# andreadiiorio/SpMV_openMP_CUDA

Measured on AMD Instinct MI355X. Metric: spmv_gflops, higher is better.
Workload: dtype f64

## Files before the change

spmv_openmp_cuda_amd/csrc/hip/tiles.hip:

```cpp
#include <hip/hip_runtime.h>
#include <cstring>
#include <cmath>
#include <chrono>
#include <rocprim/device/device_radix_sort.hpp>
#include <rocprim/device/device_scan.hpp>
#include <algorithm>
#include <vector>

#include "spmvHip.h"
#include "device_mat.hpp"

namespace spmvhip {

constexpr uint32_t PB_CBITS   = 14;
constexpr uint32_t PB_C       = 1u << PB_CBITS;
static_assert(PB_C % 1024 == 0 && PB_C * 8 <= 160 * 1024 && PB_C <= 65536, "slice width");
constexpr uint32_t PB_R_MAX   = 20000;
constexpr uint32_t PB_CUS_DEFAULT = 256;
constexpr uint32_t PB_CHUNK   = 1u << 17;
constexpr int      PB_THREADS = 1024;
constexpr uint32_t PD_WAVES   = 4;
constexpr int      PD_THREADS = PD_WAVES * 64;
constexpr size_t   PB_RESIDENT_BYTES = 288ull << 20;

struct BinMap {
    uint32_t n1 = 0, n2 = 0, a = 1, b = 1, c = 1;
    uint64_t z1 = 0, z2 = 0;
    __host__ __device__ uint32_t binOf(uint64_t row) const {
        return row < z1 ? (uint32_t)(row / a) : row < z2 ? n1 + (uint32_t)((row - z1) / b) : n1 + n2 + (uint32_t)((row - z2) / c);
    }
    __host__ __device__ uint64_t row0(uint32_t bin) const {
        return bin < n1 ? (uint64_t)bin * a : bin < n1 + n2 ? z1 + (uint64_t)(bin - n1) * b : z2 + (uint64_t)(bin - n1 - n2) * c;
    }
    __host__ __device__ uint32_t height(uint32_t bin) const { return bin < n1 ? a : bin < n1 + n2 ? b : c; }
    __host__ __device__ uint32_t maxHeight() const { uint32_t m = c; if (n1 && a > m) m = a; if (n2 && b > m) m = b; return m; }
};

struct TileFormat {
    uint32_t S = 0, B = 0, R = 0;
    BinMap    bins;
    uint64_t nnz = 0;
    void*     slab = nullptr;
    double*   val = nullptr;
    uint16_t* lcol = nullptr;
    uint16_t* lrow = nullptr;
    bool      det = false;
    uint32_t* pidx = nullptr;
    size_t    tempBytes = 0;
    uint2*    tl = nullptr;
    uint32_t  nList = 0;
    uint32_t* binPos = nullptr;
    uint32_t* waveTile = nullptr;
    uint3*    work = nullptr;
    uint32_t  nWork = 0;
    bool      ntStore = true;
    uint32_t* ready = nullptr;
    uint32_t* pushFail = nullptr;
    uint32_t  epoch = 0;
    uint32_t  cus = PB_CUS_DEFAULT;
    size_t    bytes = 0;
    spmvTilesOpts opts{0, 0, -1, 0, 0};
    uint32_t apiBins() const { return det ? (B + PD_WAVES - 1) / PD_WAVES : B; }
    uint32_t apiRows() const { return det ? PD_WAVES * bins.c : R; }
    BinMap   apiMap() const { if (!det) return bins; BinMap m; m.c = PD_WAVES * bins.c; return m; }
    uint32_t  chunk = 0;
    double    buildMs = 0;
    double    allocMs = 0;
    uint32_t* vmap = nullptr;
};

struct TileDst { double* p[SPMV_MAX_PEERS]; uint32_t n; };
struct TileSignal { uint32_t* ready; uint32_t epoch; };

namespace {

__device__ __forceinline__ uint64_t lin_block() { return (uint64_t)blockIdx.y * gridDim.x + blockIdx.x; }

struct PbPay { uint32_t vlo, vhi, row; };
static_assert(sizeof(PbPay) == 12 && alignof(PbPay) == 4, "payload layout");
__host__ __device__ __forceinline__ PbPay pb_pack(double v, uint32_t row) {
    uint64_t b;
    memcpy(&b, &v, 8);
    return PbPay{(uint32_t)b, (uint32_t)(b >> 32), row};
}
__host__ __device__ __forceinline__ double pb_value(const PbPay& e) {
    const uint64_t b = ((uint64_t)e.vhi << 32) | e.vlo;
    double v;
    memcpy(&v, &b, 8);
    return v;
}

template <typename I>
__global__ __launch_bounds__(256) void pb_payload_kernel(uint64_t M, const I* __restrict__ IRP, const uint32_t* __restrict__ JA,
                                                         const double* __restrict__ AS, uint32_t* __restrict__ keys,
                                                         PbPay* __restrict__ pay) {
    const uint64_t r = lin_block() * 4 + threadIdx.x / 64;
    if (r >= M) return;
    const uint64_t b = IRP[r], e = IRP[r + 1];
    for (uint64_t j = b + threadIdx.x % 64; j < e; j += 64) {
        const uint32_t c = JA[j];
        keys[j] = c;
        pay[j] = pb_pack(AS[j], (uint32_t)r);
    }
}

__global__ __launch_bounds__(256) void pb_bounds_kernel(
    uint64_t nnz, const PbPay* __restrict__ spay, const uint32_t* __restrict__ skeys,
    uint32_t B, BinMap bm, uint64_t nTiles, uint32_t* __restrict__ tileStart) {
    const uint64_t p = lin_block() * 256 + threadIdx.x;
    if (p >= nnz) return;
    const uint64_t t = (uint64_t)(skeys[p] >> PB_CBITS) * B + bm.binOf(spay[p].row);
    uint64_t tPrev;
    if (p == 0) tPrev = ~0ull;
    else tPrev = (uint64_t)(skeys[p - 1] >> PB_CBITS) * B + bm.binOf(spay[p - 1].row);
    if (t != tPrev)
        for (uint64_t u = tPrev + 1; u <= t; ++u) tileStart[u] = (uint32_t)p;
    if (p == nnz - 1)
        for (uint64_t u = t + 1; u <= nTiles; ++u) tileStart[u] = (uint32_t)nnz;
}

__global__ __launch_bounds__(256) void pb_lens_kernel(uint32_t S, uint32_t B, const uint32_t* __restrict__ tileStart,
                                                      uint32_t* __restrict__ lens, uint32_t* __restrict__ flags) {
    const uint64_t i = lin_block() * 256 + threadIdx.x;
    if (i >= (uint64_t)S * B) return;
    const uint32_t b = (uint32_t)(i / S), s = (uint32_t)(i % S);
    const uint64_t t = (uint64_t)s * B + b;
    const uint32_t len = tileStart[t + 1] - tileStart[t];
    lens[i] = len;
    flags[i] = len != 0;
}

__global__ __launch_bounds__(256) void pb_list_kernel(uint32_t S, uint32_t B, uint64_t nnz, const uint32_t* __restrict__ tileStart,
                                                      const uint32_t* __restrict__ lens, const uint32_t* __restrict__ bmStart,
                                                      const uint32_t* __restrict__ listIdx, uint32_t nList,
                                                      uint2* __restrict__ tl,
                                                      uint32_t* __restrict__ binPos, uint32_t* __restrict__ binTile) {
    const uint64_t i = lin_block() * 256 + threadIdx.x;
    if (i >= (uint64_t)S * B) return;
    const uint32_t b = (uint32_t)(i / S), s = (uint32_t)(i % S);
    if (lens[i]) {
        const uint64_t t = (uint64_t)s * B + b;
        tl[listIdx[i]] = make_uint2(bmStart[i], tileStart[t] - bmStart[i]);
    }
    if (s == 0) { binPos[b] = bmStart[i]; binTile[b] = listIdx[i]; }
    if (i + 1 == (uint64_t)S * B) { binPos[B] = (uint32_t)nnz; binTile[B] = nList; }
}

__global__ __launch_bounds__(256) void pb_place_kernel(
    uint64_t nnz, const PbPay* __restrict__ spay, const uint32_t* __restrict__ skeys,
    uint32_t S, uint32_t B, BinMap bm, const uint32_t* __restrict__ tileStart, const uint32_t* __restrict__ bmStart,
    double* __restrict__ val, uint16_t* __restrict__ lcol, uint16_t* __restrict__ lrow, uint32_t* __restrict__ pidx) {
    const uint64_t p = lin_block() * 256 + threadIdx.x;
    if (p >= nnz) return;
    const PbPay e = spay[p];
    const uint32_t key = skeys[p];
    const uint32_t bin = bm.binOf(e.row), slice = key >> PB_CBITS;
    val[p] = pb_value(e);
    lcol[p] = (uint16_t)(key & (PB_C - 1));
    const uint32_t within = (uint32_t)p - tileStart[(uint64_t)slice * B + bin];
    const uint32_t at = bmStart[(uint64_t)bin * S + slice] + within;
    lrow[at] = (uint16_t)(e.row - bm.row0(bin));
    if (pidx) pidx[at] = (uint32_t)p;
}

__global__ __launch_bounds__(256) void pb_fill_kernel(uint32_t* p, uint64_t n, uint32_t v) {
    const uint64_t i = lin_block() * 256 + threadIdx.x;
    if (i < n) p[i] = v;
}

__global__ __launch_bounds__(256) void pb_iota_kernel(uint64_t n, uint32_t* __restrict__ p) {
    const uint64_t i = lin_block() * 256 + threadIdx.x;
    if (i < n) p[i] = (uint32_t)i;
}
__global__ __launch_bounds__(256) void pb_invert_kernel(uint64_t n, const uint32_t* __restrict__ perm, uint32_t* __restrict__ inv) {
    const uint64_t p = lin_block() * 256 + threadIdx.x;
    if (p < n) inv[perm[p]] = (uint32_t)p;
}

typedef double   dbl2 __attribute__((ext_vector_type(2)));
typedef uint16_t ush2 __attribute__((ext_vector_type(2)));

constexpr int      P1_DEPTH = 8;
constexpr uint32_t P1_STEP  = 2 * PB_THREADS;
struct P1Regs { dbl2 a[P1_DEPTH]; ush2 c[P1_DEPTH]; };

template <bool UNIT>
__device__ __forceinline__ void p1_load(P1Regs& r, uint32_t p, uint32_t ve, const double* __restrict__ val,
                                        const uint16_t* __restrict__ lcol, double unitValue) {
#pragma unroll
    for (int u = 0; u < P1_DEPTH; ++u) {
        const uint32_t q = min(p + u * P1_STEP, ve - 2u);
        if (UNIT) r.a[u] = dbl2{unitValue, unitValue};
        else      r.a[u] = __builtin_nontemporal_load((const dbl2*)(val + q));
        r.c[u] = __builtin_nontemporal_load((const ush2*)(lcol + q));
    }
}

template <bool NT>
__device__ __forceinline__ void p1_store(const P1Regs& r, uint32_t p, uint32_t ve, const double* xs, double* __restrict__ prod) {
#pragma unroll
    for (int u = 0; u < P1_DEPTH; ++u) {
        const uint32_t q = p + u * P1_STEP;
        if (q < ve) {
            dbl2 o;
            o.x = r.a[u].x * xs[r.c[u].x]; o.y = r.a[u].y * xs[r.c[u].y];
            if (NT) __builtin_nontemporal_store(o, (dbl2*)(prod + q)); else *(dbl2*)(prod + q) = o;
        }
    }
}

template <bool NT, bool UNIT>
__global__ __launch_bounds__(PB_THREADS) void pb_expand_kernel(
    const uint3* __restrict__ work, const double* __restrict__ val, const uint16_t* __restrict__ lcol,
    const double* __restrict__ x, uint64_t N, double* __restrict__ prod, double unitValue) {
    extern __shared__ double xs[];
    const uint3 w = work[lin_block()];
    const uint32_t begin = w.y, end = w.z;
    const uint32_t vb = min(end, (begin + 63u) & ~63u);
    const uint32_t ve = vb + ((end - vb) & ~1u);
    const bool vec = ve > vb;

    uint32_t p = vb + 2 * threadIdx.x;
    P1Regs cur, nxt;
    const uint64_t col0 = (uint64_t)w.x * PB_C;
    {
        double xv[PB_C / PB_THREADS];
#pragma unroll
        for (uint32_t i = 0; i < PB_C / PB_THREADS; ++i) {
            const uint32_t k = threadIdx.x + i * PB_THREADS;
            xv[i] = (col0 + k < N) ? x[col0 + k] : 0.0;
        }
        if (vec) p1_load<UNIT>(cur, p, ve, val, lcol, unitValue);
#pragma unroll
        for (uint32_t i = 0; i < PB_C / PB_THREADS; ++i) xs[threadIdx.x + i * PB_THREADS] = xv[i];
    }
    __syncthreads();

    if (threadIdx.x < vb - begin) { const uint32_t q = begin + threadIdx.x; prod[q] = (UNIT ? unitValue : val[q]) * xs[lcol[q]]; }
    if (threadIdx.x < end - ve)   { const uint32_t q = ve + threadIdx.x;    prod[q] = (UNIT ? unitValue : val[q]) * xs[lcol[q]]; }

    if (vec) {
        constexpr uint32_t BATCH = P1_DEPTH * P1_STEP;
        for (; p < ve; p += 2 * BATCH) {
            p1_load<UNIT>(nxt, p + BATCH, ve, val, lcol, unitValue);
            p1_store<NT>(cur, p, ve, xs, prod);
            p1_load<UNIT>(cur, p + 2 * BATCH, ve, val, lcol, unitValue);
            p1_store<NT>(nxt, p + BATCH, ve, xs, prod);
        }
    }
}

constexpr int      P2_DEPTH = 8;
constexpr uint32_t P2_WAVES = PB_THREADS / 64;
constexpr uint16_t P2_NONE  = 0xFFFF;
constexpr uint32_t P2_RUNS_FLAG = 0x80000000u;
constexpr uint32_t TL_PAD   = 4;

__host__ __device__ __forceinline__ uint32_t p2_sub(uint32_t len) { return ((len + P2_WAVES - 1) / P2_WAVES + 63u) & ~63u; }

struct P2Regs { double pv[P2_DEPTH]; uint16_t rv[P2_DEPTH]; };
struct P2Cursor { uint32_t k, delta; uint2 n1, n2; };

__device__ __forceinline__ void p2_fetch(P2Regs& r, P2Cursor& c, uint32_t vbase, uint32_t we, uint32_t lane,
                                         const uint2* __restrict__ tl, const double* __restrict__ prod,
                                         const uint16_t* __restrict__ lrow) {
#pragma unroll
    for (int u = 0; u < P2_DEPTH; ++u) {
        const uint32_t vs = vbase + 64u * u;
        const uint32_t v = vs + lane, vlast = min(vs + 63u, we - 1u);
        uint32_t d = c.delta;
        while (c.n1.x <= vlast) {
            d = (v >= c.n1.x) ? c.n1.y : d;
            c.delta = c.n1.y;
            c.n1 = c.n2;
            ++c.k;
            c.n2 = tl[c.k + 2];
        }
        const uint32_t vc = min(v, we - 1u);
        r.pv[u] = prod[(uint32_t)(vc + d)];
        const uint16_t row = __builtin_nontemporal_load(lrow + vc);
        r.rv[u] = v < we ? row : P2_NONE;
    }
}

template <int D>
__device__ __forceinline__ double p2_shl(double v) {
    const uint64_t b = __double_as_longlong(v);
    const uint32_t lo = (uint32_t)__builtin_amdgcn_update_dpp(0, (int)(uint32_t)b, 0x100 + D, 0xF, 0xF, false);
    const uint32_t hi = (uint32_t)__builtin_amdgcn_update_dpp(0, (int)(uint32_t)(b >> 32), 0x100 + D, 0xF, 0xF, false);
    return __longlong_as_double(((uint64_t)hi << 32) | lo);
}

__device__ __forceinline__ uint32_t p2_prev_row(uint32_t row) {
    return (uint32_t)__builtin_amdgcn_update_dpp(-1, (int)row, 0x111, 0xF, 0xF, false);
}

__device__ __forceinline__ void p2_add_runs(double* yb, uint16_t rv, double pv, uint32_t lane) {
    const uint32_t row = rv;
    const bool follows = row == p2_prev_row(row) && row != P2_NONE;
    const uint64_t dup = __builtin_amdgcn_ballot_w64(follows);
    const uint64_t m = (~dup >> 1) >> lane;
    const uint32_t e = m ? lane + 1u + (uint32_t)__builtin_ctzll(m) : 64u;
    double v = rv != P2_NONE ? pv : 0.0;
    double t;
    t = p2_shl<1>(v); v += lane + 1 < e ? t : 0.0;
    t = p2_shl<2>(v); v += lane + 2 < e ? t : 0.0;
    t = p2_shl<4>(v); v += lane + 4 < e ? t : 0.0;
    t = p2_shl<8>(v); v += lane + 8 < e ? t : 0.0;
    if (!follows && rv != P2_NONE) atomicAdd(&yb[rv], v);
}

template <int MODE, int THREADS>
__device__ __forceinline__ void p2_finish(const double* yb, uint32_t R, uint64_t r0, uint64_t M, double* __restrict__ y,
                                          const TileDst& extra, const TileSignal& sig, uint32_t bin) {
    for (uint32_t k = threadIdx.x; k < R; k += THREADS)
        if (r0 + k < M) y[r0 + k] = yb[k];
    if (MODE == 1) {
        for (uint32_t i = 0; i < extra.n; ++i) {
            double* __restrict__ dst = extra.p[(i + bin) % extra.n];
            for (uint32_t k = threadIdx.x; k < R; k += THREADS)
                if (r0 + k < M) dst[r0 + k] = yb[k];
        }
    }
    if (MODE == 2) {
        asm volatile("s_waitcnt vmcnt(0)" ::: "memory");
        __syncthreads();
        if (threadIdx.x == 0) {
            __builtin_amdgcn_fence(__ATOMIC_RELEASE, "agent");
            asm volatile("s_waitcnt vmcnt(0)" ::: "memory");
            __hip_atomic_store(sig.ready + bin, sig.epoch, __ATOMIC_RELAXED, __HIP_MEMORY_SCOPE_AGENT);
        }
    }
}

template <int MODE>
__global__ __launch_bounds__(PB_THREADS) void pb_reduce_kernel(
    BinMap bm, uint32_t binBegin, uint32_t binEnd, uint64_t M, const uint32_t* __restrict__ binPos, const uint32_t* __restrict__ waveTile,
    const uint2* __restrict__ tl, const double* __restrict__ prod, const uint16_t* __restrict__ lrow,
    double* __restrict__ y, TileDst extra, TileSignal sig) {
    extern __shared__ double yb[];
    const uint64_t bin = binBegin + lin_block();
    if (bin >= binEnd) return;
    const uint32_t wave = (uint32_t)__builtin_amdgcn_readfirstlane((int)(threadIdx.x / 64)), lane = threadIdx.x % 64;
    const uint32_t v0 = binPos[bin], v1 = binPos[bin + 1];
    const uint32_t sub = p2_sub(v1 - v0);
    const uint32_t wb = v0 + wave * sub, we = min(v1, wb + sub);
    P2Cursor c;
    P2Regs a, b;
    bool runs = false;
    const bool busy = wave * sub < v1 - v0;
    if (busy) {
        const uint32_t wt = waveTile[bin * P2_WAVES + wave];
        runs = (wt & P2_RUNS_FLAG) != 0;
        c.k = wt & ~P2_RUNS_FLAG;
        c.delta = tl[c.k].y;
        c.n1 = tl[c.k + 1];
        c.n2 = tl[c.k + 2];
        p2_fetch(a, c, wb, we, lane, tl, prod, lrow);
    }
    const uint32_t R = bm.height((uint32_t)bin);
    for (uint32_t k = threadIdx.x; k < R; k += PB_THREADS) yb[k] = 0.0;
    __syncthreads();
    if (busy) {
        if (!runs) {
            for (uint32_t v = wb; v < we; v += 2 * P2_DEPTH * 64) {
                p2_fetch(b, c, v + P2_DEPTH * 64, we, lane, tl, prod, lrow);
#pragma unroll
                for (int u = 0; u < P2_DEPTH; ++u)
                    if (a.rv[u] != P2_NONE) atomicAdd(&yb[a.rv[u]], a.pv[u]);
                p2_fetch(a, c, v + 2 * P2_DEPTH * 64, we, lane, tl, prod, lrow);
#pragma unroll
                for (int u = 0; u < P2_DEPTH; ++u)
                    if (b.rv[u] != P2_NONE) atomicAdd(&yb[b.rv[u]], b.pv[u]);
            }
        } else {
            for (uint32_t v = wb; v < we; v += 2 * P2_DEPTH * 64) {
                p2_fetch(b, c, v + P2_DEPTH * 64, we, lane, tl, prod, lrow);
#pragma unroll
                for (int u = 0; u < P2_DEPTH; ++u) p2_add_runs(yb, a.rv[u], a.pv[u], lane);
                p2_fetch(a, c, v + 2 * P2_DEPTH * 64, we, lane, tl, prod, lrow);
#pragma unroll
                for (int u = 0; u < P2_DEPTH; ++u) p2_add_runs(yb, b.rv[u], b.pv[u], lane);
            }
        }
    }
    __syncthreads();
    p2_finish<MODE, PB_THREADS>(yb, R, bm.row0((uint32_t)bin), M, y, extra, sig, (uint32_t)bin);
}

constexpr int PD_DEPTH = 8;
struct PdStream { uint32_t idx[PD_DEPTH]; uint16_t row[PD_DEPTH]; uint32_t first; };
struct PdGather { double p[PD_DEPTH]; };

__device__ __forceinline__ void pd_stream(PdStream& s, uint32_t vb, uint32_t we, uint32_t lane, const uint32_t* __restrict__ pidx,
                                          const uint16_t* __restrict__ lrow) {
    s.first = vb;
#pragma unroll
    for (int u = 0; u < PD_DEPTH; ++u) {
        const uint32_t v = vb + 64u * u + lane, vc = min(v, we - 1u);
        s.idx[u] = __builtin_nontemporal_load(pidx + vc);
        const uint16_t r = __builtin_nontemporal_load(lrow + vc);
// ... 88 lines not shown
                const uint64_t q = i + (uint64_t)u * PUSH_THREADS;
                v[u] = *(const dbl2_t*)(src + 2 * (q < pairs ? q : i));
            }
            for (uint32_t k = 0; k < dst.n; ++k) {
                double* __restrict__ out = dst.p[(k + bin) % dst.n] + r0 + head;
#pragma unroll
                for (int u = 0; u < PUSH_DEPTH; ++u) {
                    const uint64_t q = i + (uint64_t)u * PUSH_THREADS;
                    if (q < pairs) *(dbl2_t*)(out + 2 * q) = v[u];
                }
            }
        }
        if (threadIdx.x < dst.n) {
            double* __restrict__ out = dst.p[threadIdx.x];
            if (head && r1 > r0) out[r0] = y[r0];
            if ((r1 - r0 - head) & 1) out[r1 - 1] = y[r1 - 1];
        }
        __syncthreads();
    }
}

__global__ __launch_bounds__(256) void pb_wavetile_kernel(uint32_t B, const uint32_t* __restrict__ binPos,
                                                          const uint32_t* __restrict__ binTile, const uint2* __restrict__ tl,
                                                          const uint32_t* __restrict__ dupCount, uint32_t* __restrict__ waveTile) {
    const uint64_t i = lin_block() * 256 + threadIdx.x;
    if (i >= (uint64_t)B * P2_WAVES) return;
    const uint32_t b = (uint32_t)(i / P2_WAVES), wv = (uint32_t)(i % P2_WAVES);
    const uint32_t v0 = binPos[b], v1 = binPos[b + 1];
    const uint32_t sub = p2_sub(v1 - v0);
    const uint32_t wb = v0 + wv * sub;
    uint32_t lo = binTile[b], hi = binTile[b + 1];
    if (wb >= v1 || lo >= hi) { waveTile[i] = lo; return; }
    while (hi - lo > 1) {
        const uint32_t mid = lo + (hi - lo) / 2;
        if (tl[mid].x <= wb) lo = mid; else hi = mid;
    }
    const uint32_t len = min(v1, wb + sub) - wb;
    waveTile[i] = lo | (dupCount[i] * 8 >= len ? P2_RUNS_FLAG : 0u);
}

__global__ __launch_bounds__(256) void pb_dupcount_kernel(uint32_t B, uint64_t nnz, const uint32_t* __restrict__ binPos,
                                                          const uint16_t* __restrict__ lrow, uint32_t* __restrict__ dupCount) {
    const uint64_t v = lin_block() * 256 + threadIdx.x;
    bool dup = v != 0 && v < nnz && lrow[v] == lrow[v - 1];
    uint64_t slot = 0;
    if (dup) {
        uint32_t lo = 0, hi = B;
        while (hi - lo > 1) {
            const uint32_t mid = lo + (hi - lo) / 2;
            if (binPos[mid] <= v) lo = mid; else hi = mid;
        }
        const uint32_t v0 = binPos[lo], v1 = binPos[lo + 1];
        if (v == v0) dup = false;
        else slot = (uint64_t)lo * P2_WAVES + (uint32_t)((v - v0) / p2_sub(v1 - v0));
    }
    uint64_t todo = __builtin_amdgcn_ballot_w64(dup);
    while (todo) {
        const int leader = __builtin_ctzll(todo);
        const uint64_t s0 = ((uint64_t)(uint32_t)__builtin_amdgcn_readlane((int)(uint32_t)(slot >> 32), leader) << 32) |
                            (uint32_t)__builtin_amdgcn_readlane((int)(uint32_t)slot, leader);
        const uint64_t same = __builtin_amdgcn_ballot_w64(dup && slot == s0);
        if ((int)(threadIdx.x % 64) == leader) atomicAdd(&dupCount[s0], (uint32_t)__builtin_popcountll(same));
        todo &= ~same;
    }
}

#define PB_TRY(expr) do { hipError_t e_ = (expr); if (e_ != hipSuccess) { (void)hipGetLastError(); fprintf(stderr, "libspmvhip: tiles: %s: %s\n", #expr, hipGetErrorString(e_)); return EXIT_FAILURE; } } while (0)

struct TempBuf {
    void* p = nullptr;
    ~TempBuf() { if (p) (void)hipFree(p); }
    hipError_t alloc(size_t bytes) { return hipMalloc(&p, std::max<size_t>(bytes, 1)); }
    template <typename T> T* as() { return static_cast<T*>(p); }
};

}

struct ProdWorkspace { double* p = nullptr; void* raw = nullptr; size_t cap = 0; hipEvent_t lastUse = nullptr; hipStream_t lastStream = nullptr; bool used = false, marked = false; };
static ProdWorkspace g_prod[16];

static ProdWorkspace* prodSlot() {
    int dev = 0;
    if (hipGetDevice(&dev) != hipSuccess || dev < 0 || dev >= 16) return nullptr;
    return &g_prod[dev];
}

static double* prodWorkspace(size_t n, bool grow) {
    ProdWorkspace* w = prodSlot();
    if (!w) return nullptr;
    if (n <= w->cap || !grow) return n <= w->cap ? w->p : nullptr;
    (void)hipDeviceSynchronize();
    w->used = w->marked = false;
    if (w->raw) (void)hipFree(w->raw);
    w->p = nullptr; w->raw = nullptr; w->cap = 0;
    if (hipMalloc(&w->raw, n * sizeof(double)) != hipSuccess) { w->raw = nullptr; return nullptr; }
    w->p = static_cast<double*>(w->raw);
    w->cap = n;
    return w->p;
}

static int prodHandover(hipStream_t stream) {
    ProdWorkspace* w = prodSlot();
    if (!w) return EXIT_FAILURE;
    if (w->used && w->lastStream != stream) {
        if (!w->marked || hipStreamWaitEvent(stream, w->lastUse, 0) != hipSuccess) {
            (void)hipGetLastError();
            if (hipDeviceSynchronize() != hipSuccess) return EXIT_FAILURE;
        }
    }
    w->lastStream = stream;
    w->used = true;
    w->marked = false;
    return EXIT_SUCCESS;
}

static void prodMark(hipStream_t stream) {
    ProdWorkspace* w = prodSlot();
    if (!w) return;
    hipStreamCaptureStatus cap = hipStreamCaptureStatusNone;
    if (hipStreamIsCapturing(stream, &cap) != hipSuccess || cap != hipStreamCaptureStatusNone) {
        (void)hipGetLastError();
        return;
    }
    if (!w->lastUse && hipEventCreateWithFlags(&w->lastUse, hipEventDisableTiming) != hipSuccess) { (void)hipGetLastError(); return; }
    w->marked = hipEventRecord(w->lastUse, stream) == hipSuccess;
    if (!w->marked) (void)hipGetLastError();
}

static void prodIdle() {
    if (ProdWorkspace* w = prodSlot()) w->used = w->marked = false;
}

void freeTilesWorkspace() {
    int keep = 0;
    (void)hipGetDevice(&keep);
    for (int d = 0; d < 16; ++d)
        if (g_prod[d].p || g_prod[d].lastUse) {
            (void)hipSetDevice(d);
            if (g_prod[d].raw) (void)hipFree(g_prod[d].raw);
            if (g_prod[d].lastUse) (void)hipEventDestroy(g_prod[d].lastUse);
            g_prod[d] = ProdWorkspace{};
        }
    (void)hipSetDevice(keep);
}

uint64_t tilesBinRow(const DevMat* d, const TileFormat* t, uint32_t bin) {
    if (!t) return 0;
    return bin >= t->apiBins() ? d->M : std::min<uint64_t>(d->M, t->apiMap().row0(bin));
}

void freeTiles(TileFormat* t) {
    if (!t) return;
    (void)hipFree(t->slab); (void)hipFree(t->tl); (void)hipFree(t->pidx); (void)hipFree(t->vmap);
    (void)hipFree(t->binPos); (void)hipFree(t->waveTile); (void)hipFree(t->work); (void)hipFree(t->ready);
    delete t;
}

static int buildFailed(const char* what) { (void)hipGetLastError(); fprintf(stderr, "libspmvhip: tiles: %s failed\n", what); return EXIT_FAILURE; }

static int checkTilesBuild(const DevMat* d, const spmvTilesOpts& o) {
    if (d->kind != Kind::CSR) return EXIT_FAILURE;
    if (o.deterministic && o.taper) { fprintf(stderr, "libspmvhip: tiles: the deterministic form has no tapered bins\n"); return EXIT_FAILURE; }
    if (o.rowsPerBin != 0 && (o.rowsPerBin < 64 || o.rowsPerBin > PB_R_MAX)) {
        fprintf(stderr, "libspmvhip: tiles: rowsPerBin = %u is not 0 (automatic) or 64..%u\n", o.rowsPerBin, PB_R_MAX);
        return EXIT_FAILURE;
    }
    if (o.chunk != 0 && (o.chunk < 4096 || o.chunk > (1u << 24))) {
        fprintf(stderr, "libspmvhip: tiles: chunk = %u is not 0 (automatic) or 4096..2^24\n", o.chunk);
        return EXIT_FAILURE;
    }
    const uint64_t nnz = d->NZ, N = d->N;
    if (nnz >= IRP32_LIMIT || nnz == 0) { fprintf(stderr, "libspmvhip: tiles: nnz = %lu unsupported (needs 0 < nnz < 2^32)\n", (unsigned long)nnz); return EXIT_FAILURE; }
    if ((N + PB_C - 1) / PB_C > 65535) { fprintf(stderr, "libspmvhip: tiles: %lu columns exceed 65535 slices\n", (unsigned long)N); return EXIT_FAILURE; }
    return EXIT_SUCCESS;
}

struct TileGeometry { BinMap bins; uint32_t R = 0, B = 0; };
static TileGeometry planTileBins(uint64_t M, uint32_t PB_CUS, const spmvTilesOpts& o) {
    uint32_t R = PB_R_MAX;
    const uint64_t bMin = (M + PB_R_MAX - 1) / PB_R_MAX;
    if (bMin <= 8 * PB_CUS) {
        const uint64_t b = (bMin + PB_CUS - 1) / PB_CUS * PB_CUS;
        R = (uint32_t)std::max<uint64_t>(64, ((M + b - 1) / b + 63) / 64 * 64);
        R = std::min(R, PB_R_MAX);
    }
    if (o.rowsPerBin) R = o.rowsPerBin;
    TileGeometry g;
    g.bins.c = R;
    if (o.taper != 0 && M >= (uint64_t)4 * PB_CUS * 1024) {
        const uint32_t low = std::max<uint32_t>(64, (R / 4 + 63) / 64 * 64);
        const uint64_t mid = M - (uint64_t)2 * PB_CUS * low;
        const uint64_t nb = ((mid + PB_R_MAX - 1) / PB_R_MAX + PB_CUS - 1) / PB_CUS * PB_CUS;
        const uint32_t high = std::min<uint32_t>(PB_R_MAX, (uint32_t)(((mid + nb - 1) / nb + 63) / 64 * 64));
        const uint64_t n2 = (mid + high - 1) / high;
        g.bins.n1 = PB_CUS; g.bins.a = low;
        g.bins.n2 = (uint32_t)n2; g.bins.b = high;
        g.bins.c = low;
        g.bins.z1 = (uint64_t)PB_CUS * low;
        g.bins.z2 = g.bins.z1 + n2 * high;
        if (g.bins.z2 >= M) { g.bins.n2 = (uint32_t)((M - g.bins.z1 + high - 1) / high); g.bins.z2 = g.bins.z1 + (uint64_t)g.bins.n2 * high; }
    }
    if (o.deterministic) {
        const uint32_t Rs = o.rowsPerBin ? (o.rowsPerBin + PD_WAVES - 1) / PD_WAVES
                                         : std::min<uint32_t>(PB_R_MAX / PD_WAVES / 64 * 64, std::max<uint32_t>(64, ((R + PD_WAVES - 1) / PD_WAVES + 63) / 64 * 64));
        g.bins = BinMap{};
        g.bins.c = std::max<uint32_t>(1, std::min<uint32_t>(Rs, PB_R_MAX / PD_WAVES));
    }
    g.R = g.bins.maxHeight();
    g.B = g.bins.z2 >= M ? g.bins.n1 + g.bins.n2 : g.bins.n1 + g.bins.n2 + (uint32_t)((M - g.bins.z2 + g.bins.c - 1) / g.bins.c);
    return g;
}

struct TileBuildTemps {
    TempBuf payB, sortTmp, tileStart;
    const uint32_t* skeys = nullptr;
    const PbPay* spay = nullptr;
};

static int sortIntoSlices(const DevMat* d, TileFormat* t, TileBuildTemps& tmp) {
    const uint64_t nnz = d->NZ, M = d->M, nTiles = (uint64_t)t->S * t->B;
    TempBuf &payB = tmp.payB, &sortTmp = tmp.sortTmp, &tileStart = tmp.tileStart;
    PB_TRY(hipDeviceSynchronize());
    prodIdle();
    const auto allocT0 = std::chrono::steady_clock::now();
    const size_t offLcol = (nnz * 8 + 255) / 256 * 256, offLrow = offLcol + (nnz * 2 + 255) / 256 * 256;
    const size_t slabBytes = std::max<size_t>(offLrow + nnz * 2, nnz * sizeof(PbPay));
    if (hipMalloc(&t->slab, slabBytes) || payB.alloc(nnz * sizeof(PbPay)) || tileStart.alloc((nTiles + 2) * 4))
        return buildFailed("format / temporary allocation (12 B per entry of temporaries while the format is built)");
    double* const prodBuf = prodWorkspace(nnz, true);
    if (!prodBuf || hipMalloc(&t->binPos, ((size_t)t->B + 1) * 4) || hipMalloc(&t->waveTile, (size_t)t->B * (t->det ? 1 : P2_WAVES) * 4) ||
        (t->det && hipMalloc(&t->pidx, nnz * 4)))
        return buildFailed("format allocation");
    t->allocMs = std::chrono::duration<double, std::milli>(std::chrono::steady_clock::now() - allocT0).count();
    t->val  = static_cast<double*>(t->slab);
    t->lcol = reinterpret_cast<uint16_t*>(static_cast<char*>(t->slab) + offLcol);
    t->lrow = reinterpret_cast<uint16_t*>(static_cast<char*>(t->slab) + offLrow);
    t->bytes = slabBytes + (t->det ? nnz * 4 : 0) + ((size_t)t->B + 1) * 4 + (size_t)t->B * (t->det ? 1 : P2_WAVES) * 4;
    t->tempBytes = nnz * sizeof(PbPay) + (nTiles + 2) * 4;
    uint32_t* const keysA = reinterpret_cast<uint32_t*>(prodBuf);
    PbPay* const payA = static_cast<PbPay*>(t->slab);

    withIrp(d, [&](auto irp) { hipLaunchKernelGGL((pb_payload_kernel<IrpT<decltype(irp)>>), grid2d((M + 3) / 4, 256), dim3(256), 0, nullptr, M, irp, d->JA, d->AS, keysA, payA); });
    PB_TRY(hipGetLastError());

    unsigned bits = 1;
    while ((1u << bits) < t->S) ++bits;
    rocprim::double_buffer<uint32_t> dKeys(keysA, keysA + nnz);
    rocprim::double_buffer<PbPay>    dPay(payA, payB.as<PbPay>());
    size_t tmpBytes = 0;
    PB_TRY(rocprim::radix_sort_pairs(nullptr, tmpBytes, dKeys, dPay, (size_t)nnz, PB_CBITS, PB_CBITS + bits, (hipStream_t) nullptr));
    if (sortTmp.alloc(tmpBytes)) return buildFailed("sort workspace");
    t->tempBytes += tmpBytes;
    PB_TRY(rocprim::radix_sort_pairs(sortTmp.p, tmpBytes, dKeys, dPay, (size_t)nnz, PB_CBITS, PB_CBITS + bits, (hipStream_t) nullptr));
    tmp.skeys = dKeys.current();
    if (dPay.current() == payA)
        PB_TRY(hipMemcpyAsync(payB.p, payA, nnz * sizeof(PbPay), hipMemcpyDeviceToDevice, nullptr));
    tmp.spay = payB.as<PbPay>();

    hipLaunchKernelGGL(pb_bounds_kernel, grid2d((nnz + 255) / 256, 256), dim3(256), 0, nullptr, nnz, tmp.spay, tmp.skeys, t->B, t->bins, nTiles,
                       tileStart.as<uint32_t>());
    PB_TRY(hipGetLastError());
    return EXIT_SUCCESS;
}

static int placeTiles(TileFormat* t, TileBuildTemps& tmp) {
    const uint64_t nnz = t->nnz, nTiles = (uint64_t)t->S * t->B;
    TempBuf& tileStart = tmp.tileStart;
    TempBuf lens, flags, bmStart, listIdx, scanTmp, binTile;
    if (lens.alloc(nTiles * 4) || flags.alloc(nTiles * 4) || bmStart.alloc(nTiles * 4) || listIdx.alloc(nTiles * 4) ||
        binTile.alloc(((size_t)t->B + 1) * 4))
        return buildFailed("tile-list workspace");
    t->tempBytes += nTiles * 16;
    hipLaunchKernelGGL(pb_lens_kernel, grid2d((nTiles + 255) / 256, 256), dim3(256), 0, nullptr, t->S, t->B,
                       tileStart.as<uint32_t>(), lens.as<uint32_t>(), flags.as<uint32_t>());
    size_t scanBytes = 0;
    PB_TRY(rocprim::exclusive_scan(nullptr, scanBytes, lens.as<uint32_t>(), bmStart.as<uint32_t>(), 0u, (size_t)nTiles,
                                   rocprim::plus<uint32_t>(), (hipStream_t) nullptr));
    if (scanTmp.alloc(scanBytes)) return buildFailed("scan workspace");
    PB_TRY(rocprim::exclusive_scan(scanTmp.p, scanBytes, lens.as<uint32_t>(), bmStart.as<uint32_t>(), 0u, (size_t)nTiles,
                                   rocprim::plus<uint32_t>(), (hipStream_t) nullptr));
    PB_TRY(rocprim::exclusive_scan(scanTmp.p, scanBytes, flags.as<uint32_t>(), listIdx.as<uint32_t>(), 0u, (size_t)nTiles,
                                   rocprim::plus<uint32_t>(), (hipStream_t) nullptr));
    uint32_t lastIdx = 0, lastFlag = 0;
    PB_TRY(hipMemcpy(&lastIdx, listIdx.as<uint32_t>() + nTiles - 1, 4, hipMemcpyDeviceToHost));
    PB_TRY(hipMemcpy(&lastFlag, flags.as<uint32_t>() + nTiles - 1, 4, hipMemcpyDeviceToHost));
    t->nList = lastIdx + lastFlag;
    if (t->nList >= P2_RUNS_FLAG) return buildFailed("tile list (more than 2^31 non-empty tiles)");
    if (hipMalloc(&t->tl, ((size_t)t->nList + TL_PAD) * sizeof(uint2))) return buildFailed("tile-list allocation");
    t->bytes += ((size_t)t->nList + TL_PAD) * 8;
    hipLaunchKernelGGL(pb_fill_kernel, dim3(1), dim3(256), 0, nullptr, reinterpret_cast<uint32_t*>(t->tl + t->nList), 2 * TL_PAD, 0xFFFFFFFFu);
    hipLaunchKernelGGL(pb_list_kernel, grid2d((nTiles + 255) / 256, 256), dim3(256), 0, nullptr, t->S, t->B, nnz,
                       tileStart.as<uint32_t>(), lens.as<uint32_t>(), bmStart.as<uint32_t>(), listIdx.as<uint32_t>(), t->nList,
                       t->tl, t->binPos, binTile.as<uint32_t>());
    hipLaunchKernelGGL(pb_place_kernel, grid2d((nnz + 255) / 256, 256), dim3(256), 0, nullptr, nnz, tmp.spay, tmp.skeys, t->S, t->B, t->bins,
                       tileStart.as<uint32_t>(), bmStart.as<uint32_t>(), t->val, t->lcol, t->lrow, t->pidx);
    if (t->det) {
        PB_TRY(hipMemcpyAsync(t->waveTile, binTile.p, (size_t)t->B * 4, hipMemcpyDeviceToDevice, nullptr));
    } else {
        TempBuf dupCount;
        if (dupCount.alloc((size_t)t->B * P2_WAVES * 4)) return buildFailed("run-count workspace");
        PB_TRY(hipMemsetAsync(dupCount.p, 0, (size_t)t->B * P2_WAVES * 4, nullptr));
        hipLaunchKernelGGL(pb_dupcount_kernel, grid2d((nnz + 255) / 256, 256), dim3(256), 0, nullptr, t->B, nnz, t->binPos, t->lrow,
                           dupCount.as<uint32_t>());
        hipLaunchKernelGGL(pb_wavetile_kernel, grid2d(((uint64_t)t->B * P2_WAVES + 255) / 256, 256), dim3(256), 0, nullptr, t->B,
                           t->binPos, binTile.as<uint32_t>(), t->tl, dupCount.as<uint32_t>(), t->waveTile);
        PB_TRY(hipGetLastError());
        PB_TRY(hipDeviceSynchronize());
    }
    PB_TRY(hipGetLastError());
    PB_TRY(hipDeviceSynchronize());
    return EXIT_SUCCESS;
}

static uint32_t phase1Chunk(const std::vector<uint32_t>& sliceStart, uint64_t nnz, uint32_t PB_CUS) {
    uint32_t chunk = PB_CHUNK;
    uint64_t nonEmpty = 0;
    for (size_t s = 0; s + 1 < sliceStart.size(); ++s) nonEmpty += sliceStart[s + 1] > sliceStart[s];
    const double avgLen = nonEmpty ? (double)nnz / (double)nonEmpty : 1.0;
    double bestCost = 1e300;
    const uint32_t pLo = (uint32_t)std::max(1.0, std::ceil(avgLen / 100000.0));
    const uint32_t pHi = (uint32_t)std::max((double)pLo, std::ceil(avgLen / 50000.0));
    for (uint32_t p = pLo; p <= std::min<uint32_t>(pHi, 1024); ++p) {
        const double rounds = (double)nonEmpty * p / PB_CUS;
        const double waste = (std::ceil(rounds) - rounds) / rounds;
        const double cost = 0.35 * waste + 0.1 * p * (PB_C * 8.0) / (avgLen * 18.0);
        if (cost < bestCost) { bestCost = cost; chunk = (uint32_t)std::min(16777216.0, std::ceil(avgLen / p * 1.02) + 64); }
    }
    return chunk;
}

static std::vector<uint3> interleaveSlices(const std::vector<uint3>& work) {
    std::vector<uint3> ordered;
    ordered.reserve(work.size());
    size_t i = 0;
    while (i < work.size()) {
        size_t first[9];
        int ns = 0;
        size_t j = i;
        while (j < work.size() && ns < 8) {
            first[ns++] = j;
            const uint32_t sl = work[j].x;
            while (j < work.size() && work[j].x == sl) ++j;
        }
        first[ns] = j;
        size_t maxPieces = 0;
        for (int k = 0; k < ns; ++k) maxPieces = std::max(maxPieces, first[k + 1] - first[k]);
        for (size_t pc = 0; pc < maxPieces; ++pc)
            for (int k = 0; k < ns; ++k)
                if (first[k] + pc < first[k + 1]) ordered.push_back(work[first[k] + pc]);
        i = j;
    }
    return ordered;
}

static std::vector<uint3> planPhase1Work(const std::vector<uint32_t>& sliceStart, uint32_t chunk) {
    std::vector<uint3> work;
    for (uint32_t s = 0; s + 1 < sliceStart.size(); ++s) {
        const uint32_t b0 = sliceStart[s], e0 = sliceStart[s + 1], len = e0 - b0;
        if (!len) continue;
        const uint32_t pieces = (len + chunk - 1) / chunk;
        const uint32_t piece = (len + pieces - 1) / pieces;
        uint32_t b = b0;
        for (uint32_t k = 1; k <= pieces && b < e0; ++k) {
            const uint32_t e = (k == pieces) ? e0 : std::min<uint32_t>(e0, (b0 + k * piece + 63u) & ~63u);
            if (e > b) work.push_back(make_uint3(s, b, e));
            b = e;
        }
    }
    return interleaveSlices(work);
}

static int setTilesKernelAttributes() {
    const struct { const void* kernel; int ldsBytes; } attrs[] = {
        {(const void*)pb_expand_kernel<true, false>, PB_C * 8}, {(const void*)pb_expand_kernel<false, false>, PB_C * 8},
        {(const void*)pb_expand_kernel<true, true>, PB_C * 8},  {(const void*)pb_expand_kernel<false, true>, PB_C * 8},
        {(const void*)pb_reduce_kernel<0>, PB_R_MAX * 8},       {(const void*)pb_reduce_kernel<1>, PB_R_MAX * 8},
        {(const void*)pb_reduce_kernel<2>, PB_R_MAX * 8},       {(const void*)pb_reduce_det_kernel<0>, PB_R_MAX * 8},
        {(const void*)pb_reduce_det_kernel<1>, PB_R_MAX * 8},   {(const void*)pb_reduce_det_kernel<2>, PB_R_MAX * 8}};
    for (const auto& a : attrs) PB_TRY(hipFuncSetAttribute(a.kernel, hipFuncAttributeMaxDynamicSharedMemorySize, a.ldsBytes));
    return EXIT_SUCCESS;
}

int buildTiles(DevMat* d, const spmvTilesOpts* opts) {
    const spmvTilesOpts o = opts ? *opts : spmvTilesOpts{0, 0, -1, 0, 0};
    TileFormat*& slot = d->tiles[o.deterministic != 0];
    if (slot && !opts) return EXIT_SUCCESS;
    if (checkTilesBuild(d, o)) return EXIT_FAILURE;
    if (slot) { freeTiles(slot); slot = nullptr; }
    const uint64_t nnz = d->NZ;
    TileFormat* t = new TileFormat;
    struct Guard { TileFormat*& t; ~Guard() { if (t) freeTiles(t); } } guard{t};
    {
        int dev = 0, cus = 0;
        if (hipGetDevice(&dev) == hipSuccess && hipDeviceGetAttribute(&cus, hipDeviceAttributeMultiprocessorCount, dev) == hipSuccess && cus > 0)
            t->cus = (uint32_t)cus;
    }
    hipEvent_t ev0 = nullptr, ev1 = nullptr;
    PB_TRY(hipEventCreate(&ev0));
    PB_TRY(hipEventCreate(&ev1));
    struct EvGuard { hipEvent_t a, b; ~EvGuard() { (void)hipEventDestroy(a); (void)hipEventDestroy(b); } } evGuard{ev0, ev1};
    PB_TRY(hipEventRecord(ev0, nullptr));
    const TileGeometry g = planTileBins(d->M, t->cus, o);
    t->opts = o;
    t->S = (uint32_t)((d->N + PB_C - 1) / PB_C);
    t->bins = g.bins; t->R = g.R; t->B = g.B;
    t->det = o.deterministic != 0;
    t->nnz = nnz;
    if ((uint64_t)t->S * t->B >= (1ull << 32) - 2) { fprintf(stderr, "libspmvhip: tiles: too many tiles\n"); return EXIT_FAILURE; }

    TileBuildTemps tmp;
    if (sortIntoSlices(d, t, tmp) || placeTiles(t, tmp)) return EXIT_FAILURE;

    std::vector<uint32_t> sliceStart(t->S + 1);
    PB_TRY(hipMemcpy2D(sliceStart.data(), 4, tmp.tileStart.as<uint32_t>(), (size_t)t->B * 4, 4, t->S + 1, hipMemcpyDeviceToHost));
    t->chunk = o.chunk ? o.chunk : phase1Chunk(sliceStart, nnz, t->cus);
    const std::vector<uint3> work = planPhase1Work(sliceStart, t->chunk);
    t->nWork = (uint32_t)work.size();
    PB_TRY(hipMalloc(&t->work, std::max<size_t>(work.size(), 1) * sizeof(uint3)));
    PB_TRY(hipMemcpy(t->work, work.data(), work.size() * sizeof(uint3), hipMemcpyHostToDevice));
    PB_TRY(hipDeviceSynchronize());

    if (setTilesKernelAttributes()) return EXIT_FAILURE;
    t->ntStore = o.ntStore >= 0 ? o.ntStore != 0 : nnz * 8 > PB_RESIDENT_BYTES;
    PB_TRY(hipEventRecord(ev1, nullptr));
    PB_TRY(hipEventSynchronize(ev1));
    float ms = 0;
    (void)hipEventElapsedTime(&ms, ev0, ev1);
    t->buildMs = ms;
    slot = t;
    t = nullptr;
    return EXIT_SUCCESS;
}

int tilesRefreshValues(DevMat* d, TileFormat* t, hipStream_t stream, double* mapMs, int* mapsBuilt) {
    const uint64_t nnz = t->nnz;
    if (!t->vmap) {
        const auto t0 = std::chrono::steady_clock::now();
        auto fail = [&](const char* what) {
            (void)hipGetLastError();
            fprintf(stderr, "libspmvhip: tiles: value map: %s failed\n", what);
            (void)hipStreamSynchronize(stream);
            (void)hipFree(t->vmap);
            t->vmap = nullptr;
            return EXIT_FAILURE;
        };
        if (hipMalloc(&t->vmap, std::max<uint64_t>(nnz, 1) * 4) != hipSuccess) { t->vmap = nullptr; return fail("allocation"); }
        const TileFormat* other = d->tiles[!t->det];
        if (other && other->vmap) {
            if (hipMemcpyAsync(t->vmap, other->vmap, nnz * 4, hipMemcpyDeviceToDevice, stream) != hipSuccess) return fail("copy");
        } else {
            TempBuf idx, keysOut, perm, sortTmp;
            if (idx.alloc(nnz * 4) || keysOut.alloc(nnz * 4) || perm.alloc(nnz * 4)) return fail("temporary allocation (12 B per entry)");
            hipLaunchKernelGGL(pb_iota_kernel, grid2d((nnz + 255) / 256, 256), dim3(256), 0, stream, nnz, idx.as<uint32_t>());
            unsigned bits = 1;
            while ((1u << bits) < t->S) ++bits;
            size_t tmpBytes = 0;
            if (rocprim::radix_sort_pairs(nullptr, tmpBytes, d->JA, keysOut.as<uint32_t>(), idx.as<uint32_t>(), perm.as<uint32_t>(), (size_t)nnz,
                                          PB_CBITS, PB_CBITS + bits, stream) != hipSuccess || sortTmp.alloc(tmpBytes))
                return fail("sort workspace");
            if (rocprim::radix_sort_pairs(sortTmp.p, tmpBytes, d->JA, keysOut.as<uint32_t>(), idx.as<uint32_t>(), perm.as<uint32_t>(), (size_t)nnz,
                                          PB_CBITS, PB_CBITS + bits, stream) != hipSuccess)
                return fail("sort");
            hipLaunchKernelGGL(pb_invert_kernel, grid2d((nnz + 255) / 256, 256), dim3(256), 0, stream, nnz, perm.as<uint32_t>(), t->vmap);
            if (hipGetLastError() != hipSuccess) return fail("map kernels");
        }
        if (hipStreamSynchronize(stream) != hipSuccess) return fail("synchronise");
        t->bytes += nnz * 4;
        *mapMs += std::chrono::duration<double, std::milli>(std::chrono::steady_clock::now() - t0).count();
        ++*mapsBuilt;
    }
    return enqueueScatterValues(t->val, t->vmap, nnz, d->AS, stream);
}

size_t tilesBytes(const DevMat* d) { return (d->tiles[0] ? d->tiles[0]->bytes : 0) + (d->tiles[1] ? d->tiles[1]->bytes : 0); }

void tilesInfo(const TileFormat* t, spmvTilesInfo* out) {
    memset(out, 0, sizeof *out);
    if (!t) return;
    out->nBins = t->apiBins(); out->rowsPerBin = t->apiRows(); out->nSlices = t->S; out->taper = t->bins.n1 != 0; out->ntStore = t->ntStore;
    out->chunk = t->chunk; out->buildMs = t->buildMs; out->bytes = t->bytes; out->allocMs = t->allocMs;
    out->tempBytes = t->tempBytes; out->deterministic = t->det ? 1 : 0;
}

uint32_t tilesPhase2Threads(const TileFormat* t) { return t && t->det ? (uint32_t)PD_THREADS : (uint32_t)PB_THREADS; }

void tilesShape(const TileFormat* t, uint32_t* bins, uint32_t* rowsPerBin) {
    *bins = t ? t->apiBins() : 0;
    *rowsPerBin = t ? t->apiRows() : 0;
}

int enqueueTilesExpand(const DevMat* d, const TileFormat* t, const double* x, hipStream_t stream) {
    if (!t) return EXIT_FAILURE;
    double* prod = prodWorkspace(t->nnz, true);
    if (!prod || prodHandover(stream)) return EXIT_FAILURE;
    if (t->nWork) {
#define PB_EXPAND(NT, UNIT) hipLaunchKernelGGL((pb_expand_kernel<NT, UNIT>), grid2d(t->nWork, PB_THREADS), dim3(PB_THREADS), PB_C * 8, stream, t->work, \
                                              t->val, t->lcol, x, d->N, prod, d->unitValue)
        if (d->unit) { if (t->ntStore) PB_EXPAND(true, true); else PB_EXPAND(false, true); }
        else         { if (t->ntStore) PB_EXPAND(true, false); else PB_EXPAND(false, false); }
#undef PB_EXPAND
    }
    return hipGetLastError() == hipSuccess ? EXIT_SUCCESS : EXIT_FAILURE;
}

int enqueueTilesReduce(const DevMat* d, const TileFormat* t, uint32_t binBegin, uint32_t binEnd, double* y, int nExtra, double* const* extra,
                       hipStream_t stream) {
    if (!t || binBegin > binEnd || binEnd > t->apiBins() || nExtra < 0 || nExtra > SPMV_MAX_PEERS) return EXIT_FAILURE;
    if (binBegin == binEnd) return EXIT_SUCCESS;
    const dim3 grid = grid2d((uint64_t)((binEnd - binBegin + 7) / 8) * 8, PB_THREADS);
    const double* prod = prodWorkspace(t->nnz, false);
    if (!prod || prodHandover(stream)) return EXIT_FAILURE;
    TileDst dst{};
    dst.n = (uint32_t)nExtra;
    for (int i = 0; i < nExtra; ++i) dst.p[i] = extra[i];
    const TileSignal none{nullptr, 0};
    if (t->det) {
        const size_t lds = (size_t)8 * t->apiRows();
        if (nExtra)
            hipLaunchKernelGGL(pb_reduce_det_kernel<1>, grid, dim3(PD_THREADS), lds, stream, t->bins, t->B, binBegin, binEnd, d->M, t->binPos,
                               t->pidx, prod, t->lrow, y, dst, none);
        else
            hipLaunchKernelGGL(pb_reduce_det_kernel<0>, grid, dim3(PD_THREADS), lds, stream, t->bins, t->B, binBegin, binEnd, d->M, t->binPos,
                               t->pidx, prod, t->lrow, y, dst, none);
        const bool launched = hipGetLastError() == hipSuccess;
        prodMark(stream);
        return launched ? EXIT_SUCCESS : EXIT_FAILURE;
    }
    if (nExtra)
        hipLaunchKernelGGL(pb_reduce_kernel<1>, grid, dim3(PB_THREADS), (size_t)8 * t->R, stream,
                           t->bins, binBegin, binEnd, d->M, t->binPos, t->waveTile, t->tl, prod, t->lrow, y, dst, none);
    else
        hipLaunchKernelGGL(pb_reduce_kernel<0>, grid, dim3(PB_THREADS), (size_t)8 * t->R, stream,
                           t->bins, binBegin, binEnd, d->M, t->binPos, t->waveTile, t->tl, prod, t->lrow, y, dst, none);
    const bool launched = hipGetLastError() == hipSuccess;
    prodMark(stream);
    return launched ? EXIT_SUCCESS : EXIT_FAILURE;
}

int enqueueTilesReducePush(const DevMat* d, TileFormat* t, double* y, int nExtra, double* const* extra, hipStream_t stream, hipStream_t side,
                           hipEvent_t evFork, hipEvent_t evJoin) {
    if (!t || nExtra < 1 || nExtra > SPMV_MAX_PEERS) return EXIT_FAILURE;
    const double* prod = prodWorkspace(t->nnz, true);
    if (!prod || prodHandover(stream)) return EXIT_FAILURE;
    const uint32_t nb = t->apiBins();
    if (!t->ready) {
        if (hipMalloc(&t->ready, ((size_t)nb + 1) * 4) != hipSuccess) return EXIT_FAILURE;
        if (hipMemset(t->ready, 0, ((size_t)nb + 1) * 4) != hipSuccess) return EXIT_FAILURE;
        t->pushFail = t->ready + nb;
    }
    const uint32_t epoch = ++t->epoch ? t->epoch : ++t->epoch;
    TileDst dst{};
    dst.n = (uint32_t)nExtra;
    for (int i = 0; i < nExtra; ++i) dst.p[i] = extra[i];
    const TileSignal sig{t->ready, epoch};
    if (hipEventRecord(evFork, stream) != hipSuccess || hipStreamWaitEvent(side, evFork, 0) != hipSuccess) return EXIT_FAILURE;
    hipLaunchKernelGGL(pb_push_kernel, dim3(std::min<uint32_t>(PUSH_WGS, nb)), dim3(PUSH_THREADS), 0, side, t->apiMap(), nb, d->M, t->ready,
                       epoch, y, dst, t->pushFail);
    if (t->det)
        hipLaunchKernelGGL(pb_reduce_det_kernel<2>, grid2d((uint64_t)((nb + 7) / 8) * 8, PB_THREADS), dim3(PD_THREADS), (size_t)8 * t->apiRows(), stream,
                           t->bins, t->B, 0u, nb, d->M, t->binPos, t->pidx, prod, t->lrow, y, TileDst{}, sig);
    else
        hipLaunchKernelGGL(pb_reduce_kernel<2>, grid2d((uint64_t)((t->B + 7) / 8) * 8, PB_THREADS), dim3(PB_THREADS), (size_t)8 * t->R, stream,
                           t->bins, 0u, t->B, d->M, t->binPos, t->waveTile, t->tl, prod, t->lrow, y, TileDst{}, sig);
    const bool launched = hipGetLastError() == hipSuccess;
    prodMark(stream);
    if (hipEventRecord(evJoin, side) != hipSuccess) return EXIT_FAILURE;
    return launched ? EXIT_SUCCESS : EXIT_FAILURE;
}

int tilesPushFailed(const TileFormat* t) {
    if (!t || !t->pushFail) return 0;
    uint32_t f = 0;
    if (hipMemcpy(&f, t->pushFail, 4, hipMemcpyDeviceToHost) != hipSuccess) return 1;
    return f != 0;
}

int enqueueTiles(const DevMat* d, const TileFormat* t, const double* x, double* y, hipStream_t stream) {
    if (!t) return EXIT_FAILURE;
    if (enqueueTilesExpand(d, t, x, stream)) return EXIT_FAILURE;
    return enqueueTilesReduce(d, t, 0, t->apiBins(), y, 0, nullptr, stream);
}

}
```

Baseline: 394.7.

## Make phase-1 expand kernel persistent with contiguous per-block runs of work items

Replaces the one-block-per-work-item launch of the expand kernel with a grid sized to the CU count, where each block walks a contiguous run of work items whose boundaries are cut evenly by nnz. Within a run, the block prefetches the next item's values and the next slice's x entries while finishing the current item, and restages shared-memory x only when the slice changes. This is meant to remove per-block launch, x-staging and pipeline-drain overhead, and to drop the host-side slice interleaving. The cost is a more complex control flow and possible load imbalance if items within a run vary, plus one extra device array for run offsets.

```diff
diff --git a/spmv_openmp_cuda_amd/csrc/hip/tiles.hip b/spmv_openmp_cuda_amd/csrc/hip/tiles.hip
--- a/spmv_openmp_cuda_amd/csrc/hip/tiles.hip
+++ b/spmv_openmp_cuda_amd/csrc/hip/tiles.hip
@@ -53,6 +53,8 @@
     uint32_t* waveTile = nullptr;
     uint3*    work = nullptr;
     uint32_t  nWork = 0;
+    uint32_t* runs = nullptr;
+    uint32_t  grid1 = 0;
     bool      ntStore = true;
     uint32_t* ready = nullptr;
     uint32_t* pushFail = nullptr;
@@ -187,9 +189,10 @@
 template <bool UNIT>
 __device__ __forceinline__ void p1_load(P1Regs& r, uint32_t p, uint32_t ve, const double* __restrict__ val,
                                         const uint16_t* __restrict__ lcol, double unitValue) {
+    const uint32_t hi = max(ve, 2u) - 2u;
 #pragma unroll
     for (int u = 0; u < P1_DEPTH; ++u) {
-        const uint32_t q = min(p + u * P1_STEP, ve - 2u);
+        const uint32_t q = min(p + u * P1_STEP, hi);
         if (UNIT) r.a[u] = dbl2{unitValue, unitValue};
         else      r.a[u] = __builtin_nontemporal_load((const dbl2*)(val + q));
         r.c[u] = __builtin_nontemporal_load((const ush2*)(lcol + q));
@@ -209,44 +212,83 @@
     }
 }
 
+struct P1Range { uint32_t begin, end, vb, ve; };
+__device__ __forceinline__ P1Range p1_range(const uint3 w) {
+    P1Range r;
+    r.begin = w.y; r.end = w.z;
+    r.vb = min(w.z, (w.y + 63u) & ~63u);
+    r.ve = r.vb + ((w.z - r.vb) & ~1u);
+    return r;
+}
+
+constexpr uint32_t P1_XALL = PB_C / PB_THREADS;
+constexpr uint32_t P1_XPRE = 4;
+
+template <uint32_t I0, uint32_t I1>
+__device__ __forceinline__ void p1_load_x(double (&xv)[I1 - I0], uint32_t slice, const double* __restrict__ x, uint64_t N) {
+    const double* xb = x + (uint64_t)slice * PB_C;
+    const uint32_t nIn = (uint32_t)min(N - (uint64_t)slice * PB_C, (uint64_t)PB_C);
+#pragma unroll
+    for (uint32_t i = I0; i < I1; ++i)
+        xv[i - I0] = xb[min(threadIdx.x + i * PB_THREADS, nIn - 1)];
+}
+template <uint32_t I0, uint32_t I1>
+__device__ __forceinline__ void p1_fill_x(double* xs, const double (&xv)[I1 - I0]) {
+#pragma unroll
+    for (uint32_t i = I0; i < I1; ++i) xs[threadIdx.x + i * PB_THREADS] = xv[i - I0];
+}
+
 template <bool NT, bool UNIT>
 __global__ __launch_bounds__(PB_THREADS) void pb_expand_kernel(
-    const uint3* __restrict__ work, const double* __restrict__ val, const uint16_t* __restrict__ lcol,
-    const double* __restrict__ x, uint64_t N, double* __restrict__ prod, double unitValue) {
+    const uint32_t* __restrict__ runs, const uint3* __restrict__ work, const double* __restrict__ val,
+    const uint16_t* __restrict__ lcol, const double* __restrict__ x, uint64_t N, double* __restrict__ prod, double unitValue) {
     extern __shared__ double xs[];
-    const uint3 w = work[lin_block()];
-    const uint32_t begin = w.y, end = w.z;
-    const uint32_t vb = min(end, (begin + 63u) & ~63u);
-    const uint32_t ve = vb + ((end - vb) & ~1u);
-    const bool vec = ve > vb;
-
-    uint32_t p = vb + 2 * threadIdx.x;
+    constexpr uint32_t BATCH = P1_DEPTH * P1_STEP;
+    uint32_t item = runs[blockIdx.x];
+    const uint32_t itemEnd = runs[blockIdx.x + 1];
+    if (item >= itemEnd) return;
+    const uint32_t lane2 = 2 * threadIdx.x;
+
+    uint3 w = work[item];
+    P1Range r = p1_range(w);
     P1Regs cur, nxt;
-    const uint64_t col0 = (uint64_t)w.x * PB_C;
-    {
-        double xv[PB_C / PB_THREADS];
-#pragma unroll
-        for (uint32_t i = 0; i < PB_C / PB_THREADS; ++i) {
-            const uint32_t k = threadIdx.x + i * PB_THREADS;
-            xv[i] = (col0 + k < N) ? x[col0 + k] : 0.0;
-        }
-        if (vec) p1_load<UNIT>(cur, p, ve, val, lcol, unitValue);
-#pragma unroll
-        for (uint32_t i = 0; i < PB_C / PB_THREADS; ++i) xs[threadIdx.x + i * PB_THREADS] = xv[i];
-    }
-    __syncthreads();
-
-    if (threadIdx.x < vb - begin) { const uint32_t q = begin + threadIdx.x; prod[q] = (UNIT ? unitValue : val[q]) * xs[lcol[q]]; }
-    if (threadIdx.x < end - ve)   { const uint32_t q = ve + threadIdx.x;    prod[q] = (UNIT ? unitValue : val[q]) * xs[lcol[q]]; }
-
-    if (vec) {
-        constexpr uint32_t BATCH = P1_DEPTH * P1_STEP;
-        for (; p < ve; p += 2 * BATCH) {
-            p1_load<UNIT>(nxt, p + BATCH, ve, val, lcol, unitValue);
-            p1_store<NT>(cur, p, ve, xs, prod);
-            p1_load<UNIT>(cur, p + 2 * BATCH, ve, val, lcol, unitValue);
-            p1_store<NT>(nxt, p + BATCH, ve, xs, prod);
-        }
+    double xv[P1_XPRE];
+    p1_load_x<0, P1_XPRE>(xv, w.x, x, N);
+    p1_load<UNIT>(cur, r.vb + lane2, r.ve, val, lcol, unitValue);
+    bool restage = true;
+
+    for (;;) {
+        if (restage) {
+            __syncthreads();
+            double xr[P1_XALL - P1_XPRE];
+            p1_load_x<P1_XPRE, P1_XALL>(xr, w.x, x, N);
+            p1_fill_x<0, P1_XPRE>(xs, xv);
+            p1_fill_x<P1_XPRE, P1_XALL>(xs, xr);
+            __syncthreads();
+        }
+        const bool more = item + 1 < itemEnd;
+        const uint3 wn = work[more ? item + 1 : item];
+        const P1Range rn = p1_range(wn);
+        restage = more && wn.x != w.x;
+
+        if (threadIdx.x < r.vb - r.begin) { const uint32_t q = r.begin + threadIdx.x; prod[q] = (UNIT ? unitValue : val[q]) * xs[lcol[q]]; }
+        if (threadIdx.x < r.end - r.ve)   { const uint32_t q = r.ve + threadIdx.x;    prod[q] = (UNIT ? unitValue : val[q]) * xs[lcol[q]]; }
+
+        bool last;
+        uint32_t pb = r.vb;
+        do {
+            last = pb + 2 * BATCH >= r.ve;
+            const uint32_t p = pb + lane2;
+            p1_load<UNIT>(nxt, p + BATCH, r.ve, val, lcol, unitValue);
+            p1_store<NT>(cur, p, r.ve, xs, prod);
+            if (last && restage) p1_load_x<0, P1_XPRE>(xv, wn.x, x, N);
+            const bool hand = last && more;
+            p1_load<UNIT>(cur, hand ? rn.vb + lane2 : p + 2 * BATCH, hand ? rn.ve : r.ve, val, lcol, unitValue);
+            p1_store<NT>(nxt, p + BATCH, r.ve, xs, prod);
+            pb += 2 * BATCH;
+        } while (!last);
+        if (!more) break;
+        w = wn; r = rn; ++item;
     }
 }
 
@@ -641,7 +683,7 @@
 void freeTiles(TileFormat* t) {
     if (!t) return;
     (void)hipFree(t->slab); (void)hipFree(t->tl); (void)hipFree(t->pidx); (void)hipFree(t->vmap);
-    (void)hipFree(t->binPos); (void)hipFree(t->waveTile); (void)hipFree(t->work); (void)hipFree(t->ready);
+    (void)hipFree(t->binPos); (void)hipFree(t->waveTile); (void)hipFree(t->work); (void)hipFree(t->runs); (void)hipFree(t->ready);
     delete t;
 }
 
@@ -818,32 +860,9 @@
     return chunk;
 }
 
-static std::vector<uint3> interleaveSlices(const std::vector<uint3>& work) {
-    std::vector<uint3> ordered;
-    ordered.reserve(work.size());
-    size_t i = 0;
-    while (i < work.size()) {
-        size_t first[9];
-        int ns = 0;
-        size_t j = i;
-        while (j < work.size() && ns < 8) {
-            first[ns++] = j;
-            const uint32_t sl = work[j].x;
-            while (j < work.size() && work[j].x == sl) ++j;
-        }
-        first[ns] = j;
-        size_t maxPieces = 0;
-        for (int k = 0; k < ns; ++k) maxPieces = std::max(maxPieces, first[k + 1] - first[k]);
-        for (size_t pc = 0; pc < maxPieces; ++pc)
-            for (int k = 0; k < ns; ++k)
-                if (first[k] + pc < first[k + 1]) ordered.push_back(work[first[k] + pc]);
-        i = j;
-    }
-    return ordered;
-}
-
-static std::vector<uint3> planPhase1Work(const std::vector<uint32_t>& sliceStart, uint32_t chunk) {
-    std::vector<uint3> work;
+struct Phase1Plan { std::vector<uint3> work; std::vector<uint32_t> runs; };
+static Phase1Plan planPhase1Work(const std::vector<uint32_t>& sliceStart, uint32_t chunk, uint32_t cus) {
+    std::vector<uint3> items;
     for (uint32_t s = 0; s + 1 < sliceStart.size(); ++s) {
         const uint32_t b0 = sliceStart[s], e0 = sliceStart[s + 1], len = e0 - b0;
         if (!len) continue;
@@ -852,11 +871,28 @@
         uint32_t b = b0;
         for (uint32_t k = 1; k <= pieces && b < e0; ++k) {
             const uint32_t e = (k == pieces) ? e0 : std::min<uint32_t>(e0, (b0 + k * piece + 63u) & ~63u);
-            if (e > b) work.push_back(make_uint3(s, b, e));
+            if (e > b) items.push_back(make_uint3(s, b, e));
             b = e;
         }
     }
-    return interleaveSlices(work);
+    Phase1Plan plan;
+    if (items.empty()) return plan;
+    const uint64_t nnz = items.back().z;
+    const uint32_t grid = (uint32_t)std::min<size_t>(items.size(), cus);
+    plan.runs.assign(grid + 1, 0);
+    uint32_t g = 1;
+    auto cutAt = [&](uint32_t k) { return (uint32_t)(nnz * k / grid) & ~63u; };
+    for (const uint3& it : items) {
+        uint32_t b = it.y;
+        for (; g < grid && cutAt(g) < it.z; ++g) {
+            const uint32_t c = cutAt(g);
+            if (c > b) { plan.work.push_back(make_uint3(it.x, b, c)); b = c; }
+            plan.runs[g] = (uint32_t)plan.work.size();
+        }
+        plan.work.push_back(make_uint3(it.x, b, it.z));
+    }
+    for (; g <= grid; ++g) plan.runs[g] = (uint32_t)plan.work.size();
+    return plan;
 }
 
 static int setTilesKernelAttributes() {
@@ -903,10 +939,13 @@
     std::vector<uint32_t> sliceStart(t->S + 1);
     PB_TRY(hipMemcpy2D(sliceStart.data(), 4, tmp.tileStart.as<uint32_t>(), (size_t)t->B * 4, 4, t->S + 1, hipMemcpyDeviceToHost));
     t->chunk = o.chunk ? o.chunk : phase1Chunk(sliceStart, nnz, t->cus);
-    const std::vector<uint3> work = planPhase1Work(sliceStart, t->chunk);
-    t->nWork = (uint32_t)work.size();
-    PB_TRY(hipMalloc(&t->work, std::max<size_t>(work.size(), 1) * sizeof(uint3)));
-    PB_TRY(hipMemcpy(t->work, work.data(), work.size() * sizeof(uint3), hipMemcpyHostToDevice));
+    const Phase1Plan plan = planPhase1Work(sliceStart, t->chunk, t->cus);
+    t->nWork = (uint32_t)plan.work.size();
+    t->grid1 = plan.runs.empty() ? 0 : (uint32_t)plan.runs.size() - 1;
+    PB_TRY(hipMalloc(&t->work, std::max<size_t>(plan.work.size(), 1) * sizeof(uint3)));
+    PB_TRY(hipMemcpy(t->work, plan.work.data(), plan.work.size() * sizeof(uint3), hipMemcpyHostToDevice));
+    PB_TRY(hipMalloc(&t->runs, std::max<size_t>(plan.runs.size(), 1) * sizeof(uint32_t)));
+    PB_TRY(hipMemcpy(t->runs, plan.runs.data(), plan.runs.size() * sizeof(uint32_t), hipMemcpyHostToDevice));
     PB_TRY(hipDeviceSynchronize());
 
     if (setTilesKernelAttributes()) return EXIT_FAILURE;
@@ -983,7 +1022,7 @@
     double* prod = prodWorkspace(t->nnz, true);
     if (!prod || prodHandover(stream)) return EXIT_FAILURE;
     if (t->nWork) {
-#define PB_EXPAND(NT, UNIT) hipLaunchKernelGGL((pb_expand_kernel<NT, UNIT>), grid2d(t->nWork, PB_THREADS), dim3(PB_THREADS), PB_C * 8, stream, t->work, \
+#define PB_EXPAND(NT, UNIT) hipLaunchKernelGGL((pb_expand_kernel<NT, UNIT>), dim3(t->grid1), dim3(PB_THREADS), PB_C * 8, stream, t->runs, t->work, \
                                               t->val, t->lcol, x, d->N, prod, d->unitValue)
         if (d->unit) { if (t->ntStore) PB_EXPAND(true, true); else PB_EXPAND(false, true); }
         else         { if (t->ntStore) PB_EXPAND(true, false); else PB_EXPAND(false, false); }
```

Result: faster. 411.4 (median of 6 runs) (+4.2%).
